# gcallipo/RadioDSP_SDR_RX

Measured on AMD Instinct MI355X. Metric: IQ Msamples/s through full SSB+NR chain; achieved HBM GB/s vs peak, higher is better.
Workload: dtype f32

## Files before the change

radiodsp_sdr_rx_amd/csrc/rdsp_chain.hip:

```cpp
#include <stdarg.h>
#include <stdio.h>

#include "rdsp_chain_int.h"

static thread_local char g_err[512] = "";

extern "C" void rdsp_set_error(const char *fmt, ...) {
  va_list ap;
  va_start(ap, fmt);
  vsnprintf(g_err, sizeof(g_err), fmt, ap);
  va_end(ap);
}
int chain_fail(int code, const char *fmt, ...) {
  va_list ap;
  va_start(ap, fmt);
  vsnprintf(g_err, sizeof(g_err), fmt, ap);
  va_end(ap);
  return code;
}
extern "C" const char *rdsp_last_error(void) { return g_err; }
extern "C" const char *rdsp_version(void) { return "rdsp-amd 0.2 (gfx950)"; }
extern "C" int rdsp_experimental_build(void) { return 0; }

extern "C" int rdsp_device_count(void) {
// ... 24 lines not shown
  c->n_channels = n_channels;
  c->device = device;
  c->max_blocks = max_blocks_per_call;
  c->N = cfg->fft_l;
  c->decim = decim;
  c->hop = c->N / 2;
  c->n_in = 0;
  c->old_nr_level = 15;
  c->nr_mu = rdsp_lms_mu(15);
  c->als_mu = rdsp_lms_mu(cfg->als_strength > 0 ? cfg->als_strength : 15);
  c->nr_calls = c->als_calls = 0;
  c->eng_agc_set = (cfg->agc_mode >= RDSP_AGC_FAST && cfg->agc_mode <= RDSP_AGC_SLOW) ? cfg->agc_mode : 0;
  c->fir_nat.assign(256, 0.0f);
  RC_TRY(chain_check_device(c));
  RC_TRY(chain_groups_resize(c, 1));
  GroupState &g0 = c->groups[0];
  g0.lo = cfg->flo_hz; g0.hi = cfg->fhi_hz; g0.nco_hz = cfg->nco_hz; g0.demod = cfg->demod;

  const size_t nch = (size_t)n_channels;
  HIP_TRY(alloc_zero(c->d_fir_hc, 256));
  RC_TRY(chain_planes_create(c, OPT_NONE));
  c->mid_stride = (size_t)max_blocks_per_call * RDSP_BLOCK / decim;
  HIP_TRY(alloc_zero(c->d_mid, c->mid_stride * nch));
  if (decim == 4) {
    std::vector<float> hc(256);
    if (rdsp_design_decimator(256, cfg->fir_cut_hz, cfg->fs_in, cfg->window, c->fir_nat.data(), hc.data()) != 0)
      return chain_fail(RDSP_ERR_INVALID, "decimator design failed");
    HIP_TRY(hipMemcpy(c->d_fir_hc, hc.data(), sizeof(float) * 256, hipMemcpyHostToDevice));
    std::vector<float> img(2 * 4 * (size_t)RDSP_FD_N);
    if (rdsp_fd_decimator_image(c->fir_nat.data(), RDSP_FD_N, img.data()) != 0)
      return chain_fail(RDSP_ERR_INVALID, "decimator spectra failed");
    HIP_TRY(c->d_fd_mask.alloc(img.size() / 2));
    HIP_TRY(hipMemcpy(c->d_fd_mask, img.data(), img.size() * sizeof(float), hipMemcpyHostToDevice));
    std::vector<float> rimg(2 * 4 * 256);
    rdsp_rd_decimator_image(c->fir_nat.data(), rimg.data());
    HIP_TRY(c->d_rd_mask.alloc(rimg.size() / 2));
    HIP_TRY(hipMemcpy(c->d_rd_mask, rimg.data(), rimg.size() * sizeof(float), hipMemcpyHostToDevice));
  }
  int rc = rdsp_doConvolutionalInitialize(c, nullptr);
  if (rc == RDSP_OK) rc = rdsp_reInitializeFilter(c, cfg->flo_hz, cfg->fhi_hz, nullptr);
  if (rc == RDSP_OK && cfg->demod == RDSP_DEMOD_SAM) rc = chain_ensure_sam(c);
  return rc;
}

extern "C" int rdsp_chain_create(const rdsp_chain_config_t *cfg, int n_channels, int device,
                                 int max_blocks_per_call, rdsp_chain_t **out) {
  if (!cfg || !out || n_channels <= 0 || max_blocks_per_call <= 0)
    return chain_fail(RDSP_ERR_INVALID, "rdsp_chain_create: bad argument");
  if (rdsp_plan_radix(cfg->fft_l) == 0)
    return chain_fail(RDSP_ERR_INVALID, "fft_l %d not in {256,512,1024,2048,4096}", cfg->fft_l);
  const int decim = cfg->decim <= 1 ? 1 : cfg->decim;
  if (decim != 1 && decim != 4) return chain_fail(RDSP_ERR_INVALID, "decim %d not supported (1 or 4)", cfg->decim);
  if (decim == 4 && cfg->fir_taps != 256)
    return chain_fail(RDSP_ERR_INVALID, "decimator needs 256 taps (got %d)", cfg->fir_taps);
  if (rdsp_device_count() <= 0)
    return chain_fail(RDSP_ERR_NO_DEVICE, "no HIP device: the rdsp product path has no CPU fallback");
  rdsp_chain_t *c = new rdsp_chain();
  const int rc_build = chain_build(c, cfg, n_channels, device, max_blocks_per_call, decim);
  if (rc_build != RDSP_OK) {
    rdsp_chain_destroy(c);
    return rc_build;
  }
  *out = c;
  return RDSP_OK;
}

// ... 192 lines not shown
  fp.groups = c->d_groups;
  fp.group_of = c->d_group_of;
  fp.mask_pool = c->d_mask_pool;
  fp.spectral_on = cf.spectral_nr == 2 ? 2 : (cf.spectral_nr ? 1 : 0);
  if (cf.spectral_nr == 2) {
    fp.spectral_k = 3.0f;
    fp.vad_lo = 60 * c->N / 256;
    fp.vad_hi = 120 * c->N / 256;
  } else {
    fp.spectral_k = (float)((double)cf.spectral_level * 1.5);
    fp.vad_lo = 30 * c->N / 256;
    fp.vad_hi = 180 * c->N / 256;
  }
  fp.spectral_literal = (c->spectral_literal && cf.spectral_nr == 1) ? c->spectral_literal : 0;
  fp.sin_table = c->d_sin_table;
  fp.to_mid = k.tail ? 1 : 0;
  fp.agc_on = !k.eng && cf.agc_mode != RDSP_AGC_OFF;
  fp.agc_attack = k.attack;
  fp.agc_decay = k.decay;
  fp.out_gain = k.og;
  fp.st_hist = c->d_hist;
  fp.st_prev = c->d_prev;
  fp.st_scal = c->d_scal;
  fp.out_i16 = reinterpret_cast<uint32_t *>(k.d_out);
  fp.out_stride = k.out_stride;
  fp.out_f32 = reinterpret_cast<float2 *>(k.d_out_f32);
  fp.mid_stride = c->mid_stride;
  fp.lean = (c->lean_mode < 0) ? 0 : c->lean_mode;
  fp.front_prio = k.piped ? c->front_fir_prio : 0;
  fp.fir_matrix = 0;
  fp.fir_fd = chain_fir_fd(c);
  if (c->fir_mode == -1 && fp.fir_fd == 2 && !fp.to_mid) fp.fir_fd = 3;
  fp.fd_mask = c->d_fd_mask;
  fp.rd_mask = c->d_rd_mask;
  RdspFrontPick pick;
  if (rdsp_front_pick(c->N, c->decim, &fp, &pick) == 0) c->front_name = rdsp_front_kernel_name(pick.family);
  fp.mid = (k.piped && k.slot) ? c->d_midx[k.slot - 1].p : c->d_mid.p;
  fp.mid_q = c->d_mid_q[k.piped ? k.slot : 0];
}

static int front_waits(rdsp_chain_t *c, Call &k) {
  hipStream_t stream = k.stream;
  if (k.piped && c->call_idx >= 3) HIP_TRY(hipStreamWaitEvent(stream, c->ev_tail[k.slot], 0));
  if (!k.piped && c->tail_slot >= 0) {
    HIP_TRY(hipStreamWaitEvent(stream, c->ev_tail[c->tail_slot], 0));
    c->tail_slot = -1;
  }
  if (k.timed) {
    for (int i = 0; i < 4; i++) k.ev[i] = c->ev[4 * c->ev_used + i];
    HIP_TRY(hipEventRecord(k.ev[0], stream));
  }
  bool any_dirty = false;
  for (const auto &g : c->groups) any_dirty = any_dirty || g.dirty;
  if (any_dirty && c->d_sam && c->tail_slot >= 0) HIP_TRY(hipStreamWaitEvent(stream, c->ev_tail[c->tail_slot], 0));
  return chain_groups_commit(c, stream);
}

static int launch_fronts(rdsp_chain_t *c, Call &k) {
  hipStream_t stream = k.stream;
  if (k.nsb > 1 && c->ev_front_sb[k.slot].size() < (size_t)k.nsb)
    return chain_fail(RDSP_ERR_INVALID, "sub-batch events missing (internal)");
  int e = 0;
  for (int b = 0; b < k.nsb && e == 0; b++) {
    k.fp.ch_base = b * k.sbn;
    const int count = (c->n_channels - k.fp.ch_base < k.sbn) ? c->n_channels - k.fp.ch_base : k.sbn;
    e = rdsp_launch_front(c->N, c->decim, &k.fp, count, stream);
// ... 254 lines not shown
```

radiodsp_sdr_rx_amd/csrc/rdsp_chain_groups.hip:

```cpp
#include "rdsp_chain_int.h"

static uint32_t demod_tuning_offset(int demod) {
  switch (demod) {
    case RDSP_DEMOD_LSB: return 8390u;
    case RDSP_DEMOD_USB: return 5390u;
    case RDSP_DEMOD_CW_LSB: return 7390u;
    case RDSP_DEMOD_CW_USB: return 6390u;
    case RDSP_DEMOD_AM:
    case RDSP_DEMOD_SAM: return 6890u;
    default: return 0u;
  }
}

static void group_design(rdsp_chain_t *c, GroupState &g) {
  const double fs_out = c->cfg.fs_in / (double)c->decim;
  rdsp_calc_cplx_FIR_coeffs(g.coef_I.data(), g.coef_Q.data(), c->hop + 1, g.lo, g.hi, fs_out, c->cfg.window);
}

int chain_groups_resize(rdsp_chain_t *c, int n) {
  HIP_TRY(hipDeviceSynchronize());
  if (!c->s_copy) HIP_TRY(c->s_copy.create(hipStreamNonBlocking));
  if (!c->ev_fence) HIP_TRY(c->ev_fence.create(hipEventDisableTiming));
  const size_t old = c->groups.size();
  while (c->groups.size() > (size_t)n) c->groups.pop_back();
  while (c->groups.size() < (size_t)n) c->groups.emplace_back();
  for (size_t i = 0; i < (size_t)n; i++) {
    GroupState &g = c->groups[i];
    if (i >= old) {
      if (i > 0) {
        const GroupState &g0 = c->groups[0];
        g.lo = g0.lo; g.hi = g0.hi; g.nco_hz = g0.nco_hz; g.demod = g0.demod; g.audio_filter = g0.audio_filter;
        g.coef_I = g0.coef_I; g.coef_Q = g0.coef_Q; g.mask_nat = g0.mask_nat;
        memcpy(g.iir, g0.iir, sizeof(g.iir));
      } else {
        for (int st = 0; st < 4; st++) {
          g.iir[5 * st] = 1.0f;
          g.iir[5 * st + 1] = g.iir[5 * st + 2] = g.iir[5 * st + 3] = g.iir[5 * st + 4] = 0.0f;
        }
        g.coef_I.assign(c->hop + 1, 0.0);
        g.coef_Q.assign(c->hop + 1, 0.0);
        g.mask_nat.assign(2 * (size_t)c->N, 0.0f);
      }
    }
    for (int k = 0; k < 2; k++) {
      if (!g.ev_copy[k]) HIP_TRY(g.ev_copy[k].create(hipEventDisableTiming));
      if (!g.staging[k]) HIP_TRY(g.staging[k].alloc(2 * (size_t)c->N));
    }
  }
  c->d_groups.release();
  c->d_mask_pool.release();
  HIP_TRY(alloc_zero(c->d_groups, (size_t)n));
  HIP_TRY(alloc_zero(c->d_mask_pool, 2 * (size_t)c->N * (size_t)n));
  for (auto &g : c->groups) {
    g.applied = 0;
    g.staged = -1;
    g.dirty = true;
  }
  c->fence_valid = false;
  return RDSP_OK;
}

int chain_group_stage(rdsp_chain_t *c, int gi) {
  GroupState &g = c->groups[(size_t)gi];
  const int si = g.stage_next;
  if (g.issued[si]) HIP_TRY(hipEventSynchronize(g.ev_copy[si]));
  rdsp_mask_device_image(c->cfg.filter_on ? g.mask_nat.data() : nullptr, c->N, g.staging[si]);
  const size_t img = (size_t)c->N;
  const int target = (g.staged >= 0) ? g.staged : (1 - g.applied);
  if (c->fence_valid) HIP_TRY(hipStreamWaitEvent(c->s_copy, c->ev_fence, 0));
  float2 *dst = c->d_mask_pool + ((size_t)gi * 2 + (size_t)target) * (size_t)c->N;
  HIP_TRY(hipMemcpyAsync(dst, g.staging[si], sizeof(float2) * img, hipMemcpyHostToDevice, c->s_copy));
  HIP_TRY(hipEventRecord(g.ev_copy[si], c->s_copy));
  g.issued[si] = true;
  g.stage_last = si;
  g.stage_next = si ^ 1;
  g.staged = target;
  g.dirty = true;
  return RDSP_OK;
}

static void group_record(const rdsp_chain_t *c, const GroupState &g, int gi, int buf, RdspGroup *r) {
  memset(r, 0, sizeof(*r));
  r->dphi = rdsp_nco_dphi(g.nco_hz, c->cfg.fs_in);
  r->demod = (g.demod == RDSP_DEMOD_IQ) ? RDSP_K_DEMOD_IQ
             : (g.demod == RDSP_DEMOD_AM ? RDSP_K_DEMOD_AM
                : (g.demod == RDSP_DEMOD_SAM ? RDSP_K_DEMOD_SAM : RDSP_K_DEMOD_REAL));
  float t[2];
  rdsp_nco_rot(r->dphi, 1, t); r->rot1 = make_float2(t[0], t[1]);
  rdsp_nco_rot(r->dphi, 2, t); r->rot2 = make_float2(t[0], t[1]);
  rdsp_nco_rot(r->dphi, 3, t); r->rot3 = make_float2(t[0], t[1]);
  const int nt = c->N / rdsp_plan_radix(c->N);
  rdsp_nco_rot(r->dphi, 4 * nt, t); r->rotp1 = make_float2(t[0], t[1]);
  rdsp_nco_rot(r->dphi, 8 * nt, t); r->rotp2 = make_float2(t[0], t[1]);
  rdsp_nco_rot(r->dphi, 12 * nt, t); r->rotp3 = make_float2(t[0], t[1]);
  rdsp_nco_rot(r->dphi, 256, t); r->rotq1 = make_float2(t[0], t[1]);
  rdsp_nco_rot(r->dphi, 512, t); r->rotq2 = make_float2(t[0], t[1]);
  rdsp_nco_rot(r->dphi, 768, t); r->rotq3 = make_float2(t[0], t[1]);
  r->mask_off = (uint32_t)(((size_t)gi * 2 + (size_t)buf) * (size_t)c->N);
  r->dphi_hist = g.has_dev_dphi ? g.dev_dphi : r->dphi;
  rdsp_nco_rot(r->dphi_hist, 1, t); r->roth1 = make_float2(t[0], t[1]);
  rdsp_nco_rot(r->dphi_hist, 2, t); r->roth2 = make_float2(t[0], t[1]);
  rdsp_nco_rot(r->dphi_hist, 3, t); r->roth3 = make_float2(t[0], t[1]);
  rdsp_nco_rot(r->dphi_hist, 12 * nt, t); r->rothp3 = make_float2(t[0], t[1]);
}

int chain_groups_commit(rdsp_chain_t *c, hipStream_t stream) {
  for (size_t i = 0; i < c->groups.size(); i++) {
    GroupState &g = c->groups[i];
    if (!g.dirty) continue;
    int buf = g.applied;
    if (g.staged >= 0) {
      HIP_TRY(hipStreamWaitEvent(stream, g.ev_copy[g.stage_last], 0));
      buf = g.staged;
    }
    RdspGroup r;
    group_record(c, g, (int)i, buf, &r);
    int e = rdsp_launch_group_store(c->d_groups + i, &r, stream);
    if (e != 0) return launch_failed("group record update failed", e);
    g.applied = buf;
    g.staged = -1;
    g.dirty = (r.dphi_hist != r.dphi);
    g.has_dev_dphi = true;
    g.dev_dphi = r.dphi;
  }
  return RDSP_OK;
}

int chain_check_group(const rdsp_chain_t *c, int group) {
  if (!c || group < 0 || (size_t)group >= c->groups.size())
    return chain_fail(RDSP_ERR_INVALID, "group %d out of range", group);
  return RDSP_OK;
}

static int group_initialize(rdsp_chain_t *c, int gi) {
  GroupState &g = c->groups[(size_t)gi];
  if (rdsp_init_filter_mask(g.mask_nat.data(), g.coef_I.data(), g.coef_Q.data(), c->N) != 0)
    return chain_fail(RDSP_ERR_INVALID, "init_filter_mask failed");
  return chain_group_stage(c, gi);
}

extern "C" int rdsp_doConvolutionalInitialize(rdsp_chain_t *c, void *stream) {
  (void)stream;
  if (!c) return RDSP_ERR_INVALID;
  RC_TRY(chain_check_device(c));
  for (size_t i = 0; i < c->groups.size(); i++) RC_TRY(group_initialize(c, (int)i));
  return RDSP_OK;
// ... 217 lines not shown
```

radiodsp_sdr_rx_amd/csrc/rdsp_chain_int.h:

```cpp
#ifndef RDSP_CHAIN_INT_H
#define RDSP_CHAIN_INT_H

#include <hip/hip_runtime.h>
#include <math.h>
#include <string.h>

#include <array>
#include <deque>
#include <vector>

#include "rdsp_dev.h"
#include "rdsp_host.h"
#include "rdsp_kernels.h"

using namespace rdsp_dev;

int chain_fail(int code, const char *fmt, ...) __attribute__((format(printf, 2, 3)));
#define NEED(c) do { if (!(c)) return RDSP_ERR_INVALID; } while (0)
#define TO_ENGINE(c, call) do { NEED(c); if ((c)->engine) return (call); } while (0)

static inline int launch_failed(const char *what, int e) {
  return chain_fail(RDSP_ERR_HIP, "%s: %s", what, hipGetErrorString((hipError_t)e));
}
static inline hipError_t push_event(std::deque<Event> &pool, unsigned flags) {
  pool.emplace_back();
  const hipError_t e = pool.back().create(flags);
  if (e != hipSuccess) pool.pop_back();
  return e;
}

struct GroupState {
  double lo = 0.0, hi = 0.0, nco_hz = 0.0;
  int demod = RDSP_DEMOD_USB, audio_filter = RDSP_AUDIO_2700;
  std::vector<double> coef_I, coef_Q;
  std::vector<float> mask_nat;
  int applied = 0;
  int staged = -1;
  bool dirty = true;
  bool has_dev_dphi = false;
  uint32_t dev_dphi = 0;
  Event ev_copy[2];
  PinnedBuf<float> staging[2];
  bool issued[2] = {false, false};
  int stage_next = 0, stage_last = 0;
  float iir[20];
  bool iir_dirty = true;
};
struct rdsp_chain {
  rdsp_chain_config_t cfg;
  int n_channels, device, max_blocks;
  int N, decim, hop;
  uint64_t n_in;
  int old_nr_level;
  float nr_mu, als_mu;
  long nr_calls, als_calls;
  std::vector<float> fir_nat;
  std::deque<GroupState> groups;
  std::vector<uint16_t> group_of;
  DevBuf<RdspGroup> d_groups;
  DevBuf<uint16_t> d_group_of;
  DevBuf<float2> d_mask_pool;
  Stream s_copy;
  Event ev_fence;
  bool fence_valid = false;
  DevBuf<float> d_fir_hc;
  DevBuf<float2> d_fd_mask;
  DevBuf<float2> d_rd_mask;
  DevBuf<float> d_sin_table;
  int spectral_literal = 0;
  rdsp_engine_t *engine = nullptr;
  rdsp_preproc_t *pre = nullptr;
  DevBuf<int16_t> d_engine_io;
  int nlms_energy_running = 0;
  DevBuf<uint32_t> d_hist;
  DevBuf<float2> d_prev;
  DevBuf<float> d_scal;
  DevBuf<float> d_nr_w, d_nr_prev, d_nr_energy;
  DevBuf<float> d_als_w, d_als_prev, d_als_energy;
  DevBuf<uint32_t> d_status;
  DevBuf<float> d_mid;
  size_t mid_stride = 0;
  DevBuf<float> d_mid_q[3], d_sam;
  int pipe_on = 0;
  Stream s_tail;
  Stream s_mid;
  Event ev_mid[3];
  Event ev_front[3], ev_tail[3], ev_misc;
  int sub_batch = 4096;
  std::deque<Event> ev_front_sb[3];
  DevBuf<float> d_midx[2];
  long call_idx = 0;
  int tail_slot = -1;
  int timing_on = 0;
  std::deque<Event> ev;
  std::vector<int> ev_has_tail;
  size_t ev_used = 0;
  int lean_mode = -1;
  int fir_mode = -1;
  int front_fir_prio = 2, tail_prio = 2;
  int tail_lpc = 100;
// ... 53 lines not shown
```

radiodsp_sdr_rx_amd/csrc/rdsp_design.c:

```c
#include "rdsp_host.h"

#include <math.h>
#include <stdlib.h>
#include <string.h>
#ifdef _OPENMP
#include <omp.h>
#endif

static const double kPi = 3.14159265358979323846;

static double cosine_sum_window(int id, int i, int n) {
  static const double rows[3][4] = {
      {0.35875, 0.48829, 0.14128, 0.01168},
      {0.355768, 0.487396, 0.144232, 0.012604},
      {0.3635819, 0.4891775, 0.1365995, 0.0106411}
  };
  const double t = 2.0 * kPi * (double)i / (double)(n - 1);
  if (id == 3) return cos(0.5 * t);
  if (id == 4) return 0.5 * (1.0 - cos(t));
  const double *a = rows[id == 1 ? 0 : (id == 2 ? 1 : 2)];
  return a[0] - a[1] * cos(t) + a[2] * cos(2.0 * t) - a[3] * cos(3.0 * t);
}

void rdsp_calc_cplx_FIR_coeffs(double *coeffs_I, double *coeffs_Q, int numCoeffs, double FLoCut,
// ... 136 lines not shown
  for (int c = 0; c < 4; c++)
    for (int kp = 0; kp < 64; kp++) hc[c * 64 + kp] = h_nat[4 * kp + c];
  free(ti);
  return 0;
}

int rdsp_fd_decimator_image(const float *h_nat, int fft_l, float *image) {
  const int P = rdsp_plan_radix(fft_l);
  if (P == 0 || fft_l < 128) return -1;
  const int nt = fft_l / P;
  const double inv_n = 1.0 / (double)fft_l;
  for (int r = 0; r < 4; r++) {
    double g[65];
    for (int k = 0; k <= 64; k++) {
      const int t = 4 * k - r;
      g[k] = (t >= 0 && t < 256) ? (double)h_nat[t] : 0.0;
    }
    for (int t = 0; t < nt; t++)
      for (int e = 0; e < P; e++) {
        const int bin = rdsp_bin_of_pos(fft_l, t * P + e);
        double re = 0.0, im = 0.0;
        for (int k = 0; k <= 64; k++) {
          const int m = (int)(((long long)bin * k) % fft_l);
          const double a = -2.0 * kPi * (double)m / (double)fft_l;
          re += g[k] * cos(a);
          im += g[k] * sin(a);
        }
        const size_t o = (size_t)r * (size_t)fft_l + (size_t)e * (size_t)nt + (size_t)t;
        image[2 * o] = (float)(re * inv_n);
        image[2 * o + 1] = (float)(im * inv_n);
      }
  }
  return 0;
}

int rdsp_rd_decimator_image(const float *h_nat, float *image) {
  const int n = 256;
  for (int r = 0; r < 4; r++) {
    double g[65];
    for (int k = 0; k <= 64; k++) {
      const int t = 4 * k - r;
      g[k] = (t >= 0 && t < 256) ? (double)h_nat[t] : 0.0;
    }
    for (int bin = 0; bin < n; bin++) {
      double re = 0.0, im = 0.0;
      for (int k = 0; k <= 64; k++) {
        const int m = (bin * k) % n;
        const double a = -2.0 * kPi * (double)m / (double)n;
        re += g[k] * cos(a);
        im += g[k] * sin(a);
      }
      const size_t o = (size_t)r * n + (size_t)(bin >> 4) * 16 + (size_t)(bin & 15);
      image[2 * o] = (float)(re / n);
      image[2 * o + 1] = (float)(im / n);
    }
  }
  return 0;
}

void rdsp_biquad_design(int kind, double freq, double q, double fs, float *coef5) {
  const double w0 = 2.0 * kPi * freq / fs;
  const double cs = cos(w0), alpha = sin(w0) / (2.0 * q);
  const double a0 = 1.0 + alpha;
  double num[3];
  if (kind == 0) { num[1] = 1.0 - cs; num[0] = num[2] = 0.5 * num[1]; }
  else if (kind == 1) { num[1] = -(1.0 + cs); num[0] = num[2] = -0.5 * num[1]; }
// ... 172 lines not shown
```

radiodsp_sdr_rx_amd/csrc/rdsp_front_fd.hip:

```cpp
#include <stdlib.h>

#include "rdsp_front_frame.h"
#include "rdsp_front_launch.h"

using namespace rdsp;

namespace {

template <int N, int P, bool Q4>
struct FrontFdLds {
  static constexpr int NW = N / P / 64;
  static constexpr int RING_N = Q4 ? QUAD_RING : (NW == 1 ? 1024 : 4096);
  static constexpr int WB_N0 = FftPlan<N, P>::WB > NW * FftPlan<RDSP_FD_N, RDSP_FD_P>::WB ? FftPlan<N, P>::WB : NW * FftPlan<RDSP_FD_N, RDSP_FD_P>::WB;
  static constexpr int WB_N = (Q4 && QUAD_WB > WB_N0) ? QUAD_WB : WB_N0;
  static constexpr int RED_N = 64;
  static constexpr int NBCOL_N = NW > 1 ? NW * 64 : 0;
  static constexpr int NBACC_N = NW > 1 ? 64 : 0;
  static constexpr int NBS_BYTES = NW > 1 ? 16 : 0;
  static constexpr size_t RING = 0;
  static constexpr size_t WB = RING + RING_N * sizeof(float2);
  static constexpr size_t RED = WB + WB_N * sizeof(float2);
  static constexpr size_t NBCOL = RED + RED_N * sizeof(float);
  static constexpr size_t NBACC = NBCOL + NBCOL_N * sizeof(uint4);
  static constexpr size_t NBS = NBACC + NBACC_N * sizeof(float);
  static constexpr size_t BYTES = NBS + NBS_BYTES;
};

template <int N, int P, bool LEAN, bool PRE, bool Q4 = false, int VC = RDSP_FD_P - 1>
__global__ void __launch_bounds__(N / P, 2) rdsp_front_fd_kernel(RdspFrontParams p) {
  using PL = FftPlan<N, P>;
  constexpr int ND = RDSP_FD_N, PD = RDSP_FD_P;
  using PLD = FftPlan<ND, PD>;
  constexpr int NT = PL::NT;
  constexpr int H = N / 2;
  constexpr int PH = P / 2;
  constexpr int VAL = 64 * VC;
  constexpr int NC = VC + 1;
  static_assert(VC == PD - 1 || VC == 4, "448-sample frames or one granule per frame");
  constexpr int NW = NT / 64;
  constexpr bool QUAD = Q4;
  static_assert(!Q4 || N == 256, "the four-frame form exists for FFT_L 256");
  using LY = FrontFdLds<N, P, Q4>;
  constexpr int RING = LY::RING_N;
  constexpr bool SAME = (N == ND && P == PD);
  static_assert((NT == 64 || NT == 256) && PLD::NT == 64, "one or four waves per channel, one per decimator frame");
  static_assert(QUAD || H - 1 + NW * VAL <= RING, "ring holds a round's outputs behind an unfinished hop");
  static_assert(!QUAD || H + (4 * H - 64) + VAL <= QUAD_HOPS * H, "the overlap hop and what is unconsumed (< 4 hops, in steps of 64) survive a frame's seven columns");

  extern __shared__ __attribute__((aligned(16))) unsigned char smem_raw[];
  float2 *ring = reinterpret_cast<float2 *>(smem_raw + LY::RING);
  float2 *wb = reinterpret_cast<float2 *>(smem_raw + LY::WB);
  float *red = reinterpret_cast<float *>(smem_raw + LY::RED);

  const bool SWAP_IQ = PRE && p.swap_iq != 0;
  const bool NB_ON = PRE && p.nb_on != 0;
  uint4 *nbcol = reinterpret_cast<uint4 *>(smem_raw + LY::NBCOL);
  float *nbacc = reinterpret_cast<float *>(smem_raw + LY::NBACC);
  float *nbs = reinterpret_cast<float *>(smem_raw + LY::NBS);
  const int tid = threadIdx.x;
  const int lane = tid & 63, wave = tid >> 6;
  float2 *wbd = wb + wave * PLD::WB;
  const size_t ch = (size_t)p.ch_base + blockIdx.x;
  const uint32_t *iq = p.iq + ch * p.in_stride;
  RdspGroup G;
  const uint32_t gi = p.group_of ? (uint32_t)__builtin_amdgcn_readfirstlane((int)p.group_of[ch]) : 0u;
  {
    const uint32_t *gw = reinterpret_cast<const uint32_t *>(p.groups + gi);
    uint32_t r[32];
#pragma unroll
    for (int i = 0; i < 32; i++) r[i] = (i < 30) ? (uint32_t)__builtin_amdgcn_readfirstlane((int)gw[i]) : 0u;
    G = __builtin_bit_cast(RdspGroup, r);
  }
  const int total = p.n_chunks * 256;

  const __amdgpu_buffer_rsrc_t iq_rsrc = __builtin_amdgcn_make_buffer_rsrc(const_cast<uint32_t *>(iq), 0, 16 * total, 0x00020000);
  auto ld_quad = [&](int q) {
    typedef int v4i __attribute__((ext_vector_type(4)));
    const v4i v = __builtin_amdgcn_raw_buffer_load_b128(iq_rsrc, 16 * q, 0, NW == 1 ? 2 : 0);
    return make_uint4((uint32_t)v.x, (uint32_t)v.y, (uint32_t)v.z, (uint32_t)v.w);
  };
  uint4 rq[NC];
#pragma unroll
  for (int j = 0; j < NC; j++) {
    const int q = wave * VAL - 64 + lane + 64 * j;
    if (q < 0) rq[j] = *reinterpret_cast<const uint4 *>(p.st_hist + ch * 256 + 4 * lane);
    else rq[j] = ld_quad(q);
  }

  Twiddles<N, P, LEAN> tw;
  LdsBases<N, P, false> lb;
  if constexpr (!QUAD) {
    tw.init(tid);
    make_lds_bases<N, P, false>(tid, lb);
  }
  Twiddles<256, 16, LEAN> tw16;
  LdsBases<256, 16, false> lb16;
  if constexpr (QUAD) {
    tw16.init(lane & 15);
    make_lds_bases<256, 16, false>(lane & 15, lb16);
  }
  const int mbase = 16 * (lane & 3) + 4 * ((lane >> 2) & 3);
  Twiddles<ND, PD, false> twd_own;
  LdsBases<ND, PD, false> lbd_own;
// ... 106 lines not shown
        swap0 = RDSP_LATE(swap_hist) != 0;
      }
      dphi_hist = RDSP_GROUP_LATE_U32(gi, dphi_hist);
    }
    const bool fold = !PRE || p.scale_i == p.scale_q, fold0 = !PRE || si0 == sq0;
    const float gph = fold ? p.scale_i : 1.0f, gph0 = fold0 ? si0 : 1.0f;
    const float sxi = fold ? 1.0f : p.scale_i, sxq = fold ? 1.0f : p.scale_q;
    const float sxi0 = fold0 ? 1.0f : si0, sxq0 = fold0 ? 1.0f : sq0;
    float2 pj[NC];
    {
      float2 b1u = make_float2(1.f, 0.f);
      if (G.dphi != 0u) b1u = nco_phasor_alu((nq + 256u) * G.dphi);
      const float2 b1 = make_float2(b1u.x * gph, b1u.y * gph);
      if (hist && dphi_hist != G.dphi) {
        const float2 d = (dphi_hist != 0u) ? nco_phasor_alu(nq * dphi_hist) : make_float2(1.f, 0.f);
        pj[0] = make_float2(d.x * gph0, d.y * gph0);
      } else if (PRE && gph0 != gph) {
        pj[0] = cmulc_uniform(make_float2(b1u.x * gph0, b1u.y * gph0), G.rotq1);
      } else {
        pj[0] = cmulc_uniform(b1, G.rotq1);
      }
      pj[1] = b1;
      if constexpr (PD > 2) pj[2] = cmul_pinned_u(b1, G.rotq1);
      if constexpr (PD > 3) pj[3] = cmul_pinned_u(b1, G.rotq2);
#pragma unroll
      for (int j = 4; j < NC; j++) pj[j] = cmul_pinned_u(pj[j - 3], G.rotq3);
    }

    float2 acc[PD];
#pragma unroll
    for (int r = 0; r < 4; r++) {
      float2 gm[PD];
      {
        const float2 *mp = p.fd_mask + (size_t)r * ND;
        asm volatile("" : "+s"(mp));
        const auto gp = as_global(mp);
#pragma unroll
        for (int e = 0; e < PD; e++) gm[e] = gp[e * 64 + lane];
      }
      float2 v[PD];
#pragma unroll
      for (int j = NC; j < PD; j++) v[j] = make_float2(0.f, 0.f);
#pragma unroll
      for (int j = 0; j < NC; j++) {
        uint32_t w = (r == 0) ? rq[j].x : (r == 1) ? rq[j].y : (r == 2) ? rq[j].z : rq[j].w;
        if (j == 0 ? swap0 : SWAP_IQ) w = __builtin_amdgcn_alignbit(w, w, 16);
        float2 x = make_float2((float)(int16_t)(w & 0xFFFFu), (float)(int16_t)(w >> 16));
        if constexpr (PRE) x = make_float2(x.x * (j == 0 ? sxi0 : sxi), x.y * (j == 0 ? sxq0 : sxq));
        float2 ph = pj[j];
        if (r > 0) {
          const float2 rr = (r == 1) ? G.rot1 : (r == 2) ? G.rot2 : G.rot3;
          if (j == 0) {
            float2 r0 = rr;
            if (hist) r0 = (r == 1) ? RDSP_GROUP_LATE_F2(gi, roth1) : (r == 2) ? RDSP_GROUP_LATE_F2(gi, roth2) : RDSP_GROUP_LATE_F2(gi, roth3);
            ph = cmul_pinned_u(ph, r0);
          } else {
            ph = cmul_pinned_u(ph, rr);
          }
        }
        v[j] = cmul_pinned(x, ph);
      }
      if (r == 3) {
        if constexpr (NW == 1) rq[0] = rq[VC];
#pragma unroll
        for (int j = (NW == 1 ? 1 : 0); j < NC; j++) {
          const int q = (fr + NW) * VAL - 64 + lane + 64 * j;
          rq[j] = ld_quad(q);
        }
      }
      {
        float2 twp[PD - 1];
        twd.template get<0>(twp);
        fwd_pass0_store<ND, PD>(lbd, v, wbd, twp);
      }
      wg_sync<1>();
      fwd_mid_all<ND, PD, 1, PLD::NP - 1, false>(lbd, wbd, twd, wsync);
      fwd_pass_last<ND, PD>(lbd, v, wbd);
      wg_sync<1>();
#pragma unroll
      for (int e = 0; e < PD; e++) acc[e] = (r == 0) ? cmul(v[e], gm[e]) : cmac(acc[e], v[e], gm[e]);
    }
    inv_pass_last<ND, PD>(lbd, acc, wbd);
    wg_sync<1>();
// ... 53 lines not shown
      consumed += H;
    }
  }

  float2 *const st_prev = RDSP_LATE(st_prev);
  uint32_t *const st_hist = RDSP_LATE(st_hist);
  float *const st_scal = RDSP_LATE(st_scal);
  if constexpr (QUAD) {
    const int hp = rhop == 0 ? QUAD_HOPS - 1 : rhop - 1;
#pragma unroll
    for (int j = 0; j < PH; j++) st_prev[ch * H + tid + j * NT] = ring[hp * QUAD_PITCH + tid + j * NT];
  } else {
#pragma unroll
    for (int j = 0; j < PH; j++) st_prev[ch * H + tid + j * NT] = vprev[j];
  }
  if (tid < 64 && !(NB_ON && NW > 1))
    *reinterpret_cast<uint4 *>(st_hist + ch * 256 + 4 * tid) =
        NB_ON ? hist_save : *reinterpret_cast<const uint4 *>(iq + 4 * (total - 64 + tid));
  if (tid == 0) {
    st_scal[ch * 4 + 0] = nfloor;
    if (!p.to_mid) st_scal[ch * 4 + 1] = agc_g;
    st_scal[ch * 4 + 2] = am_dc;
    if (NB_ON) st_scal[ch * 4 + 3] = (NW > 1) ? nbs[0] : nb_level;
  }
}

inline size_t granule_form_lds_pad(int to_mid) {
  static const long env = getenv("RDSP_FD_LDS_PAD") ? atol(getenv("RDSP_FD_LDS_PAD")) : -1;
  if (env >= 0) return (size_t)env;
  (void)to_mid;
  return 0;
}

template <int N, int P, bool LEAN, bool PRE, bool Q4, int VC>
int launch_fd(const RdspFrontParams *p, int n_channels, hipStream_t stream) {
  constexpr size_t lds = FrontFdLds<N, P, Q4>::BYTES;
  static_assert(!Q4 || lds <= 48 * 1024, "no raised dynamic-LDS limit needed");
  if constexpr (lds > 48 * 1024) {
    int e = ensure_lds_limit<&rdsp_front_fd_kernel<N, P, LEAN, PRE, Q4, VC>>(lds);
    if (e != 0) return e;
  }
  size_t ask = lds;
  if constexpr (!Q4 && lds <= 16 * 1024) ask = lds + granule_form_lds_pad(p->to_mid);
  hipLaunchKernelGGL((rdsp_front_fd_kernel<N, P, LEAN, PRE, Q4, VC>), dim3(n_channels), dim3(N / P), ask, stream, *p);
  return (int)hipGetLastError();
}

template <int N, int P, bool LEAN, bool Q4>
constexpr bool fd_instance = (LEAN || P != 16) && (!Q4 || N == 256);

}

int rdsp::front_fd_launch(int fft_l, const RdspFrontPick &k, const RdspFrontParams *p, int n_channels, hipStream_t stream) {
  if (k.frame != 4 && k.frame != RDSP_FD_P - 1) return (int)hipErrorInvalidValue;
  return with_front_plan(fft_l, (int)hipErrorInvalidValue, [&](auto plan) {
    return with_flag(k.lean, [&](auto lean) {
      return with_flag(k.pre, [&](auto pre) {
        return with_flag(k.q4, [&](auto q4) {
          constexpr int N = decltype(plan)::N, P = decltype(plan)::P;
          constexpr bool LEAN = decltype(lean)::value, PRE = decltype(pre)::value, Q4 = decltype(q4)::value;
          if constexpr (fd_instance<N, P, LEAN, Q4>)
            return k.frame == 4 ? launch_fd<N, P, LEAN, PRE, Q4, 4>(p, n_channels, stream)
                                : launch_fd<N, P, LEAN, PRE, Q4, RDSP_FD_P - 1>(p, n_channels, stream);
          else return (int)hipErrorInvalidValue;
        });
      });
    });
  });
}
```

radiodsp_sdr_rx_amd/csrc/rdsp_host.h:

```cpp
#ifndef RDSP_HOST_H
#define RDSP_HOST_H

#include "../../include/rdsp.h"

#ifdef __cplusplus
extern "C" {
#endif

int rdsp_plan_radix(int fft_l);
int rdsp_bin_of_pos(int fft_l, int i);
void rdsp_mask_device_image(const float *mask_nat, int fft_l, float *image);
int rdsp_design_decimator(int ntaps, double cut_hz, double fs, int window, float *h_nat, float *hc);
int rdsp_fd_decimator_image(const float *h_nat, int fft_l, float *image);
int rdsp_rd_decimator_image(const float *h_nat, float *image);
uint32_t rdsp_nco_dphi(double hz, double fs);
void rdsp_nco_rot(uint32_t dphi, int k, float *out2);
float rdsp_lms_mu(int strength);
void rdsp_sam_constants(double fs_out, float *g1, float *g2, float *wmin, float *wmax);
void rdsp_set_error(const char *fmt, ...);
void rdsp_arm_sin_table(float *tab513);
void rdsp_q15_twiddles(int n, uint32_t *out);
const uint16_t *rdsp_sqrt_guess_table(void);
float rdsp_q15_read(const uint16_t *output, unsigned int bins, unsigned int binNumber);
float rdsp_q15_read_range(const uint16_t *output, unsigned int bins, unsigned int binFirst, unsigned int binLast, int inclusive);
void rdsp_host_fft(double *re, double *im, int n);

#ifdef __cplusplus
}
#endif
#endif
```

radiodsp_sdr_rx_amd/csrc/rdsp_kernels.h:

```cpp
#ifndef RDSP_KERNELS_H
#define RDSP_KERNELS_H

#include <hip/hip_runtime.h>
#include <stdint.h>

#define RDSP_BLOCK 128
#define RDSP_LMS_TAPS 96
#define RDSP_FD_N 512
#define RDSP_FD_P 8
#define RDSP_XP 84

enum { RDSP_K_DEMOD_IQ = 0, RDSP_K_DEMOD_REAL = 1, RDSP_K_DEMOD_AM = 2, RDSP_K_DEMOD_SAM = 3 };

struct RdspGroup {
  uint32_t dphi;
  int32_t demod;
  float2 rot1, rot2, rot3;
  float2 rotp1, rotp2, rotp3;
  uint32_t mask_off;
  uint32_t dphi_hist;
  float2 roth1, roth2, roth3;
  float2 rothp3;
  float2 rotq1, rotq2, rotq3;
  uint32_t pad[2];
};

struct RdspFrontParams {
  const uint32_t *iq;
  size_t in_stride;
  int n_chunks;
  uint32_t n0;
  const RdspGroup *groups;
  const uint16_t *group_of;
  float scale_i, scale_q;
  int swap_iq;
  float scale_i_hist, scale_q_hist;
  int swap_hist;
  int nb_on;
  float nb_thr;
  const float *fir_hc;
  const float2 *mask_pool;
  int spectral_on;
  float spectral_k;
  int spectral_literal;
  const float *sin_table;
  int vad_lo, vad_hi;
  int to_mid;
  int lean;
  int fir_matrix;
  int fir_fd;
  const float2 *fd_mask;
  const float2 *rd_mask;
  int front_prio;
  int agc_on;
  float agc_attack, agc_decay;
  float out_gain;
  uint32_t *st_hist;
  float2 *st_prev;
  float *st_scal;
  uint32_t *out_i16;
  size_t out_stride;
  float2 *out_f32;
  float *mid;
  float *mid_q;
  size_t mid_stride;
  int ch_base;
};

enum { RDSP_FRONT_DIRECT = 0, RDSP_FRONT_FD = 1, RDSP_FRONT_RD = 2 };
struct RdspFrontPick {
  int family;
  int radix;
  int lean;
  int pre;
  int q4;
  int frame;
};

struct RdspSamParams {
  float *mid;
  const float *mid_q;
  size_t mid_stride;
  int n_channels;
  int n_samples;
  const RdspGroup *groups;
  const uint16_t *group_of;
  float g1, g2, wmin, wmax;
  float *st_sam;
};

struct RdspTailParams {
  const float *mid;
  size_t mid_stride;
  int n_channels;
  int ch_base;
  int n_blocks;
  int nr_on, als_mode;
  int nr_mode;
  int prio;
  int energy_running;
// ... 41 lines not shown
  int prio;
  EngineAgcSet agc;
  float curve[130];
};

struct RdspBiquadParams {
  float *buf;
  size_t stride;
  const int16_t *in16;
  size_t stride16;
  int step16;
  int16_t *out16;
  size_t ostride16;
  int ostep16;
  int n_channels;
  int ch_base;
  int n_samples;
  const float *coef;
  const uint16_t *set_of;
  float *state;
  const int *icoef;
  int n_stages;
  int *istate;
};

#ifdef __cplusplus
extern "C" {
#endif
int rdsp_launch_biquad(const RdspBiquadParams *p, hipStream_t stream);
int rdsp_launch_biquad_coef_store(float *dst, const float *coef20, hipStream_t stream);
int rdsp_launch_front(int fft_l, int decim, const RdspFrontParams *p, int n_channels,
                      hipStream_t stream);
int rdsp_front_pick(int fft_l, int decim, const RdspFrontParams *p, RdspFrontPick *pick);
const char *rdsp_front_kernel_name(int family);
int rdsp_launch_tail(const RdspTailParams *p, int lanes_per_channel, hipStream_t stream);
int rdsp_launch_sam(const RdspSamParams *p, hipStream_t stream);
int rdsp_launch_tail_engine(const RdspTailEngineParams *p, hipStream_t stream);
void rdsp_tail_engine_constants(RdspTailEngineParams *p, int agc_set);
int rdsp_launch_group_store(RdspGroup *dst, const RdspGroup *val, hipStream_t stream);
int rdsp_launch_iq_slip(const uint32_t *in, size_t in_stride, uint32_t *out, size_t out_stride, const uint32_t *carry_in,
                        size_t carry_stride, uint32_t *carry_out, int n_samples, int slip, int n_channels, hipStream_t stream);
int rdsp_launch_q15_to_float(const int16_t *src, float *dst, size_t n, hipStream_t stream);
int rdsp_launch_float_to_q15(const float *src, int16_t *dst, size_t n, hipStream_t stream);
size_t rdsp_front_lds_bytes(int fft_l, int decim);
#ifdef __cplusplus
}
#endif

#endif
```

radiodsp_sdr_rx_amd/csrc/rdsp_kernels.hip:

```cpp
#include <stdlib.h>
#include <string.h>

#include "rdsp_front.h"
#include "rdsp_front_launch.h"

using namespace rdsp;

namespace {

struct RdspGroupWords { uint32_t w[32]; };
__global__ void rdsp_group_store_kernel(uint32_t *dst, RdspGroupWords v) { dst[threadIdx.x] = v.w[threadIdx.x]; }

__global__ void __launch_bounds__(256) rdsp_iq_slip_kernel(const uint32_t *in, size_t in_stride, uint32_t *out,
                                                           size_t out_stride, const uint32_t *carry_in, size_t carry_stride,
                                                           uint32_t *carry_out, int n_quads, int slip) {
  const int q = blockIdx.x * 256 + threadIdx.x;
  const size_t ch = blockIdx.y;
  if (q >= n_quads) return;
  const uint32_t *src = in + ch * in_stride;
  const uint4 w = *reinterpret_cast<const uint4 *>(src + 4 * (size_t)q);
  const uint32_t p = (q == 0) ? carry_in[ch * carry_stride] : src[4 * (size_t)q - 1];
  const uint32_t lo = 0x0000FFFFu;
  uint4 r;
  if (slip > 0) {
// ... 19 lines not shown
}

extern "C" int rdsp_front_pick(int fft_l, int decim, const RdspFrontParams *p, RdspFrontPick *pick) {
  if (decim != 1 && decim != 4) return (int)hipErrorInvalidValue;
  RdspFrontPick k = {};
  k.radix = with_front_plan(fft_l, 0, [](auto plan) { return decltype(plan)::P; });
  if (!k.radix) return (int)hipErrorInvalidValue;
  k.lean = k.radix == 16 || p->lean;
  const bool hist_differs = p->swap_hist != p->swap_iq || p->scale_i_hist != p->scale_i || p->scale_q_hist != p->scale_q;
  k.pre = p->nb_on || p->swap_iq || hist_differs || p->scale_i != p->scale_q;
  const bool one_hop_frames = fft_l == 256 && !p->to_mid;
  if (decim == 4 && p->fir_fd) {
    if (p->fir_fd >= 3 && !p->nb_on) {
      if (!p->rd_mask) return (int)hipErrorInvalidValue;
      if (p->fir_fd == 4) return (int)hipErrorNotSupported;
      k.family = RDSP_FRONT_RD;
      k.lean = k.radix >= 8;
      k.frame = 128;
      k.q4 = one_hop_frames;
    } else {
      static const bool no_quad = getenv("RDSP_NO_QUAD") && atoi(getenv("RDSP_NO_QUAD")) != 0;
      k.family = RDSP_FRONT_FD;
      k.frame = (p->fir_fd == 2 || p->fir_fd == 3) ? 4 : RDSP_FD_P - 1;
      k.q4 = one_hop_frames && !no_quad;
    }
  } else {
    if (p->fir_matrix) return (int)hipErrorNotSupported;
    k.family = RDSP_FRONT_DIRECT;
  }
  *pick = k;
  return 0;
}

extern "C" const char *rdsp_front_kernel_name(int family) {
  return family == RDSP_FRONT_RD ? "rdsp_front_rd_kernel" : (family == RDSP_FRONT_FD ? "rdsp_front_fd_kernel" : "rdsp_front_kernel");
}

extern "C" int rdsp_launch_front(int fft_l, int decim, const RdspFrontParams *p, int n_channels,
                                 hipStream_t stream) {
  RdspFrontPick k;
  const int e = rdsp_front_pick(fft_l, decim, p, &k);
  if (e != 0) return e;
  switch (k.family) {
    case RDSP_FRONT_RD: return front_rd_launch(fft_l, k, p, n_channels, stream);
    case RDSP_FRONT_FD: return front_fd_launch(fft_l, k, p, n_channels, stream);
    default: return front_direct_launch(fft_l, decim, k, p, n_channels, stream);
  }
}

extern "C" int rdsp_launch_group_store(RdspGroup *dst, const RdspGroup *val, hipStream_t stream) {
  static_assert(sizeof(RdspGroup) == 128, "group record is 32 dwords");
  RdspGroupWords v;
  memcpy(&v, val, sizeof(v));
  hipLaunchKernelGGL(rdsp_group_store_kernel, dim3(1), dim3(32), 0, stream, reinterpret_cast<uint32_t *>(dst), v);
  return (int)hipGetLastError();
}

extern "C" int rdsp_launch_iq_slip(const uint32_t *in, size_t in_stride, uint32_t *out, size_t out_stride,
                                   const uint32_t *carry_in, size_t carry_stride, uint32_t *carry_out, int n_samples,
                                   int slip, int n_channels, hipStream_t stream) {
  const int nq = n_samples / 4;
  hipLaunchKernelGGL(rdsp_iq_slip_kernel, dim3((nq + 255) / 256, n_channels), dim3(256), 0, stream, in, in_stride, out,
                     out_stride, carry_in, carry_stride, carry_out, nq, slip);
  return (int)hipGetLastError();
}

// ... 15 lines not shown
```

Measured before the change: 241,900.

## Precompute per-group NCO-rotated decimator spectra to drop in-kernel phase rotation

```diff
diff --git a/radiodsp_sdr_rx_amd/csrc/rdsp_chain.hip b/radiodsp_sdr_rx_amd/csrc/rdsp_chain.hip
--- a/radiodsp_sdr_rx_amd/csrc/rdsp_chain.hip
+++ b/radiodsp_sdr_rx_amd/csrc/rdsp_chain.hip
@@ -80,6 +80,7 @@
       return chain_fail(RDSP_ERR_INVALID, "decimator spectra failed");
     HIP_TRY(c->d_fd_mask.alloc(img.size() / 2));
     HIP_TRY(hipMemcpy(c->d_fd_mask, img.data(), img.size() * sizeof(float), hipMemcpyHostToDevice));
+    c->fd_img = std::move(img);
     std::vector<float> rimg(2 * 4 * 256);
     rdsp_rd_decimator_image(c->fir_nat.data(), rimg.data());
     HIP_TRY(c->d_rd_mask.alloc(rimg.size() / 2));
@@ -338,6 +339,7 @@
   fp.fir_fd = chain_fir_fd(c);
   if (c->fir_mode == -1 && fp.fir_fd == 2 && !fp.to_mid) fp.fir_fd = 3;
   fp.fd_mask = c->d_fd_mask;
+  fp.rot_pool = c->d_rot_pool;
   fp.rd_mask = c->d_rd_mask;
   RdspFrontPick pick;
   if (rdsp_front_pick(c->N, c->decim, &fp, &pick) == 0) c->front_name = rdsp_front_kernel_name(pick.family);
diff --git a/radiodsp_sdr_rx_amd/csrc/rdsp_chain_groups.hip b/radiodsp_sdr_rx_amd/csrc/rdsp_chain_groups.hip
--- a/radiodsp_sdr_rx_amd/csrc/rdsp_chain_groups.hip
+++ b/radiodsp_sdr_rx_amd/csrc/rdsp_chain_groups.hip
@@ -12,6 +12,7 @@
   }
 }
 
+static const size_t kRotImg = 4 * (size_t)RDSP_FD_N;
 static void group_design(rdsp_chain_t *c, GroupState &g) {
   const double fs_out = c->cfg.fs_in / (double)c->decim;
   rdsp_calc_cplx_FIR_coeffs(g.coef_I.data(), g.coef_Q.data(), c->hop + 1, g.lo, g.hi, fs_out, c->cfg.window);
@@ -49,12 +50,21 @@
   }
   c->d_groups.release();
   c->d_mask_pool.release();
+  c->d_rot_pool.release();
   HIP_TRY(alloc_zero(c->d_groups, (size_t)n));
   HIP_TRY(alloc_zero(c->d_mask_pool, 2 * (size_t)c->N * (size_t)n));
+  const bool rot = c->decim == 4 && n <= RDSP_FD_ROT_GROUPS;
+  if (rot) HIP_TRY(alloc_zero(c->d_rot_pool, 2 * kRotImg * (size_t)n));
   for (auto &g : c->groups) {
     g.applied = 0;
     g.staged = -1;
     g.dirty = true;
+    g.rot_applied = 0;
+    g.rot_valid = false;
+    for (int k = 0; k < 2 && rot; k++) {
+      if (!g.ev_rot[k]) HIP_TRY(g.ev_rot[k].create(hipEventDisableTiming));
+      if (!g.rot_staging[k]) HIP_TRY(g.rot_staging[k].alloc(2 * kRotImg));
+    }
   }
   c->fence_valid = false;
   return RDSP_OK;
@@ -97,11 +107,30 @@
   rdsp_nco_rot(r->dphi, 512, t); r->rotq2 = make_float2(t[0], t[1]);
   rdsp_nco_rot(r->dphi, 768, t); r->rotq3 = make_float2(t[0], t[1]);
   r->mask_off = (uint32_t)(((size_t)gi * 2 + (size_t)buf) * (size_t)c->N);
+  r->rot_off = c->d_rot_pool ? (uint32_t)(((size_t)gi * 2 + (size_t)g.rot_applied) * kRotImg) : 0u;
   r->dphi_hist = g.has_dev_dphi ? g.dev_dphi : r->dphi;
   rdsp_nco_rot(r->dphi_hist, 1, t); r->roth1 = make_float2(t[0], t[1]);
   rdsp_nco_rot(r->dphi_hist, 2, t); r->roth2 = make_float2(t[0], t[1]);
   rdsp_nco_rot(r->dphi_hist, 3, t); r->roth3 = make_float2(t[0], t[1]);
   rdsp_nco_rot(r->dphi_hist, 12 * nt, t); r->rothp3 = make_float2(t[0], t[1]);
+}
+
+static int group_stage_rot(rdsp_chain_t *c, int gi, uint32_t dphi, hipStream_t stream) {
+  GroupState &g = c->groups[(size_t)gi];
+  const int si = g.rot_next;
+  if (g.rot_issued[si]) HIP_TRY(hipEventSynchronize(g.ev_rot[si]));
+  rdsp_fd_rot_image(c->fd_img.data(), RDSP_FD_N, dphi, g.rot_staging[si]);
+  const int target = g.rot_valid ? 1 - g.rot_applied : g.rot_applied;
+  if (c->fence_valid) HIP_TRY(hipStreamWaitEvent(stream, c->ev_fence, 0));
+  float2 *dst = c->d_rot_pool + ((size_t)gi * 2 + (size_t)target) * kRotImg;
+  HIP_TRY(hipMemcpyAsync(dst, g.rot_staging[si], sizeof(float2) * kRotImg, hipMemcpyHostToDevice, stream));
+  HIP_TRY(hipEventRecord(g.ev_rot[si], stream));
+  g.rot_issued[si] = true;
+  g.rot_next = si ^ 1;
+  g.rot_applied = target;
+  g.rot_dphi = dphi;
+  g.rot_valid = true;
+  return RDSP_OK;
 }
 
 int chain_groups_commit(rdsp_chain_t *c, hipStream_t stream) {
@@ -112,6 +141,10 @@
     if (g.staged >= 0) {
       HIP_TRY(hipStreamWaitEvent(stream, g.ev_copy[g.stage_last], 0));
       buf = g.staged;
+    }
+    if (c->d_rot_pool) {
+      const uint32_t dphi = rdsp_nco_dphi(g.nco_hz, c->cfg.fs_in);
+      if (!g.rot_valid || g.rot_dphi != dphi) RC_TRY(group_stage_rot(c, (int)i, dphi, stream));
     }
     RdspGroup r;
     group_record(c, g, (int)i, buf, &r);
diff --git a/radiodsp_sdr_rx_amd/csrc/rdsp_chain_int.h b/radiodsp_sdr_rx_amd/csrc/rdsp_chain_int.h
--- a/radiodsp_sdr_rx_amd/csrc/rdsp_chain_int.h
+++ b/radiodsp_sdr_rx_amd/csrc/rdsp_chain_int.h
@@ -43,6 +43,13 @@
   PinnedBuf<float> staging[2];
   bool issued[2] = {false, false};
   int stage_next = 0, stage_last = 0;
+  int rot_applied = 0;
+  bool rot_valid = false;
+  uint32_t rot_dphi = 0;
+  Event ev_rot[2];
+  PinnedBuf<float> rot_staging[2];
+  bool rot_issued[2] = {false, false};
+  int rot_next = 0;
   float iir[20];
   bool iir_dirty = true;
 };
@@ -66,6 +73,8 @@
   DevBuf<float> d_fir_hc;
   DevBuf<float2> d_fd_mask;
   DevBuf<float2> d_rd_mask;
+  std::vector<float> fd_img;
+  DevBuf<float2> d_rot_pool;
   DevBuf<float> d_sin_table;
   int spectral_literal = 0;
   rdsp_engine_t *engine = nullptr;
diff --git a/radiodsp_sdr_rx_amd/csrc/rdsp_design.c b/radiodsp_sdr_rx_amd/csrc/rdsp_design.c
--- a/radiodsp_sdr_rx_amd/csrc/rdsp_design.c
+++ b/radiodsp_sdr_rx_amd/csrc/rdsp_design.c
@@ -192,6 +192,20 @@
       }
   }
   return 0;
+}
+
+void rdsp_fd_rot_image(const float *image, int fft_l, uint32_t dphi, float *out) {
+  for (int r = 0; r < 4; r++) {
+    const uint32_t ph = dphi * (uint32_t)r;
+    const double a = 2.0 * kPi * (double)ph / 4294967296.0;
+    const double c = cos(a), s = -sin(a);
+    for (int k = 0; k < fft_l; k++) {
+      const size_t o = 2 * ((size_t)r * (size_t)fft_l + (size_t)k);
+      const double re = (double)image[o], im = (double)image[o + 1];
+      out[o] = r ? (float)(re * c - im * s) : image[o];
+      out[o + 1] = r ? (float)(re * s + im * c) : image[o + 1];
+    }
+  }
 }
 
 int rdsp_rd_decimator_image(const float *h_nat, float *image) {
diff --git a/radiodsp_sdr_rx_amd/csrc/rdsp_front_fd.hip b/radiodsp_sdr_rx_amd/csrc/rdsp_front_fd.hip
--- a/radiodsp_sdr_rx_amd/csrc/rdsp_front_fd.hip
+++ b/radiodsp_sdr_rx_amd/csrc/rdsp_front_fd.hip
@@ -26,7 +26,7 @@
   static constexpr size_t BYTES = NBS + NBS_BYTES;
 };
 
-template <int N, int P, bool LEAN, bool PRE, bool Q4 = false, int VC = RDSP_FD_P - 1>
+template <int N, int P, bool LEAN, bool PRE, bool Q4 = false, int VC = RDSP_FD_P - 1, bool ROTG = false>
 __global__ void __launch_bounds__(N / P, 2) rdsp_front_fd_kernel(RdspFrontParams p) {
   using PL = FftPlan<N, P>;
   constexpr int ND = RDSP_FD_N, PD = RDSP_FD_P;
@@ -68,7 +68,7 @@
     const uint32_t *gw = reinterpret_cast<const uint32_t *>(p.groups + gi);
     uint32_t r[32];
 #pragma unroll
-    for (int i = 0; i < 32; i++) r[i] = (i < 30) ? (uint32_t)__builtin_amdgcn_readfirstlane((int)gw[i]) : 0u;
+    for (int i = 0; i < 32; i++) r[i] = (i < 31) ? (uint32_t)__builtin_amdgcn_readfirstlane((int)gw[i]) : 0u;
     G = __builtin_bit_cast(RdspGroup, r);
   }
   const int total = p.n_chunks * 256;
@@ -241,7 +241,7 @@
     for (int r = 0; r < 4; r++) {
       float2 gm[PD];
       {
-        const float2 *mp = p.fd_mask + (size_t)r * ND;
+        const float2 *mp = ROTG ? p.rot_pool + G.rot_off + (size_t)r * ND : p.fd_mask + (size_t)r * ND;
         asm volatile("" : "+s"(mp));
         const auto gp = as_global(mp);
 #pragma unroll
@@ -257,7 +257,12 @@
         float2 x = make_float2((float)(int16_t)(w & 0xFFFFu), (float)(int16_t)(w >> 16));
         if constexpr (PRE) x = make_float2(x.x * (j == 0 ? sxi0 : sxi), x.y * (j == 0 ? sxq0 : sxq));
         float2 ph = pj[j];
-        if (r > 0) {
+        if constexpr (ROTG) {
+          if (r > 0 && j == 0 && hist && dphi_hist != G.dphi) {
+            ph = cmul_pinned_u(ph, (r == 1) ? RDSP_GROUP_LATE_F2(gi, roth1) : (r == 2) ? RDSP_GROUP_LATE_F2(gi, roth2) : RDSP_GROUP_LATE_F2(gi, roth3));
+            ph = cmulc_uniform(ph, (r == 1) ? RDSP_GROUP_LATE_F2(gi, rot1) : (r == 2) ? RDSP_GROUP_LATE_F2(gi, rot2) : RDSP_GROUP_LATE_F2(gi, rot3));
+          }
+        } else if (r > 0) {
           const float2 rr = (r == 1) ? G.rot1 : (r == 2) ? G.rot2 : G.rot3;
           if (j == 0) {
             float2 r0 = rr;
@@ -377,17 +382,17 @@
   return 0;
 }
 
-template <int N, int P, bool LEAN, bool PRE, bool Q4, int VC>
+template <int N, int P, bool LEAN, bool PRE, bool Q4, int VC, bool ROTG>
 int launch_fd(const RdspFrontParams *p, int n_channels, hipStream_t stream) {
   constexpr size_t lds = FrontFdLds<N, P, Q4>::BYTES;
   static_assert(!Q4 || lds <= 48 * 1024, "no raised dynamic-LDS limit needed");
   if constexpr (lds > 48 * 1024) {
-    int e = ensure_lds_limit<&rdsp_front_fd_kernel<N, P, LEAN, PRE, Q4, VC>>(lds);
+    int e = ensure_lds_limit<&rdsp_front_fd_kernel<N, P, LEAN, PRE, Q4, VC, ROTG>>(lds);
     if (e != 0) return e;
   }
   size_t ask = lds;
   if constexpr (!Q4 && lds <= 16 * 1024) ask = lds + granule_form_lds_pad(p->to_mid);
-  hipLaunchKernelGGL((rdsp_front_fd_kernel<N, P, LEAN, PRE, Q4, VC>), dim3(n_channels), dim3(N / P), ask, stream, *p);
+  hipLaunchKernelGGL((rdsp_front_fd_kernel<N, P, LEAN, PRE, Q4, VC, ROTG>), dim3(n_channels), dim3(N / P), ask, stream, *p);
   return (int)hipGetLastError();
 }
 
@@ -405,8 +410,11 @@
           constexpr int N = decltype(plan)::N, P = decltype(plan)::P;
           constexpr bool LEAN = decltype(lean)::value, PRE = decltype(pre)::value, Q4 = decltype(q4)::value;
           if constexpr (fd_instance<N, P, LEAN, Q4>)
-            return k.frame == 4 ? launch_fd<N, P, LEAN, PRE, Q4, 4>(p, n_channels, stream)
-                                : launch_fd<N, P, LEAN, PRE, Q4, RDSP_FD_P - 1>(p, n_channels, stream);
+            return with_flag(rdsp_front_pick_rotg(p) != 0, [&](auto rotg) {
+              constexpr bool ROTG = decltype(rotg)::value;
+              return k.frame == 4 ? launch_fd<N, P, LEAN, PRE, Q4, 4, ROTG>(p, n_channels, stream)
+                                  : launch_fd<N, P, LEAN, PRE, Q4, RDSP_FD_P - 1, ROTG>(p, n_channels, stream);
+            });
           else return (int)hipErrorInvalidValue;
         });
       });
diff --git a/radiodsp_sdr_rx_amd/csrc/rdsp_host.h b/radiodsp_sdr_rx_amd/csrc/rdsp_host.h
--- a/radiodsp_sdr_rx_amd/csrc/rdsp_host.h
+++ b/radiodsp_sdr_rx_amd/csrc/rdsp_host.h
@@ -12,6 +12,7 @@
 void rdsp_mask_device_image(const float *mask_nat, int fft_l, float *image);
 int rdsp_design_decimator(int ntaps, double cut_hz, double fs, int window, float *h_nat, float *hc);
 int rdsp_fd_decimator_image(const float *h_nat, int fft_l, float *image);
+void rdsp_fd_rot_image(const float *image, int fft_l, uint32_t dphi, float *out);
 int rdsp_rd_decimator_image(const float *h_nat, float *image);
 uint32_t rdsp_nco_dphi(double hz, double fs);
 void rdsp_nco_rot(uint32_t dphi, int k, float *out2);
diff --git a/radiodsp_sdr_rx_amd/csrc/rdsp_kernels.h b/radiodsp_sdr_rx_amd/csrc/rdsp_kernels.h
--- a/radiodsp_sdr_rx_amd/csrc/rdsp_kernels.h
+++ b/radiodsp_sdr_rx_amd/csrc/rdsp_kernels.h
@@ -22,7 +22,8 @@
   float2 roth1, roth2, roth3;
   float2 rothp3;
   float2 rotq1, rotq2, rotq3;
-  uint32_t pad[2];
+  uint32_t rot_off;
+  uint32_t pad;
 };
 
 struct RdspFrontParams {
@@ -65,7 +66,9 @@
   float *mid_q;
   size_t mid_stride;
   int ch_base;
+  const float2 *rot_pool;
 };
+#define RDSP_FD_ROT_GROUPS 64
 
 enum { RDSP_FRONT_DIRECT = 0, RDSP_FRONT_FD = 1, RDSP_FRONT_RD = 2 };
 struct RdspFrontPick {
@@ -173,6 +176,7 @@
 int rdsp_launch_front(int fft_l, int decim, const RdspFrontParams *p, int n_channels,
                       hipStream_t stream);
 int rdsp_front_pick(int fft_l, int decim, const RdspFrontParams *p, RdspFrontPick *pick);
+int rdsp_front_pick_rotg(const RdspFrontParams *p);
 const char *rdsp_front_kernel_name(int family);
 int rdsp_launch_tail(const RdspTailParams *p, int lanes_per_channel, hipStream_t stream);
 int rdsp_launch_sam(const RdspSamParams *p, hipStream_t stream);
diff --git a/radiodsp_sdr_rx_amd/csrc/rdsp_kernels.hip b/radiodsp_sdr_rx_amd/csrc/rdsp_kernels.hip
--- a/radiodsp_sdr_rx_amd/csrc/rdsp_kernels.hip
+++ b/radiodsp_sdr_rx_amd/csrc/rdsp_kernels.hip
@@ -75,6 +75,8 @@
   return 0;
 }
 
+extern "C" int rdsp_front_pick_rotg(const RdspFrontParams *p) { return p->rot_pool != nullptr; }
+
 extern "C" const char *rdsp_front_kernel_name(int family) {
   return family == RDSP_FRONT_RD ? "rdsp_front_rd_kernel" : (family == RDSP_FRONT_FD ? "rdsp_front_fd_kernel" : "rdsp_front_kernel");
 }
```

After: 245,800 (median of 6 runs). 1.02x the previous value.
